# AaltoML/nonstationary-audio-gp

Measured on AMD Instinct MI355X. Metric: audio samples/sec filtered+smoothed (state dim 146, per EP sweep), higher is better.
Workload: dtype f64

## Files before the change

nonstationary-audio-gp_amd/csrc/nagp_api.hip:

```cpp
#include "nagp_inst.hpp"
#include "nagp_recon.hpp"
#include "nagp_fbsample.hpp"
#include "nagp_epsample.hpp"
#include "nagp_slowfb.hpp"
#include "nagp_nmf.hpp"
#include "nagp_pstft.hpp"
#include "nagp_segp.hpp"
#include "nagp_gppad.hpp"
#include "nagp_gppad_lap.hpp"
#include "nagp_tridiag.hpp"
#include "nagp_nmf_temp.hpp"
#include "nagp_sebf.hpp"
#include "../../include/nagp.h"

NAGP_LIST_ALL(extern template __global__)
NAGP_LIST_FBSAMPLE(extern template __global__)
NAGP_LIST_EPSAMPLE(extern template __global__)
NAGP_LIST_SLOWFB(extern template __global__)
NAGP_LIST_NMF(extern template __global__)
NAGP_LIST_PSTFT(extern template __global__)
NAGP_LIST_SEGP(extern template __global__)
NAGP_LIST_GPPAD(extern template __global__)
NAGP_LIST_GPPAD_CAS(extern template __global__)
NAGP_LIST_GPPAD_LAP(extern template __global__)
// ... 146 lines not shown
  int mfma_sp = 0;
  int big_sp = 0;
  int gain768 = 0;
  int gain_mfma = 0;
  int gain_inv = 0;
  double* d_ainv = nullptr;
  size_t gbuf_doubles = 0;
  MfmaPar mpar{};
  size_t lds_mfma = 0;
  int hph_lds = 0, sta_f = 0, sta_ep = 0, DG_f = 1, DG_ep = 1, cache_f = 0, cache_ep = 0, kb_f = 16;
  bool want_PS = false;
  bool need_PF = false;
  MomSrc src_all{};
  int src_f = 0, src_ep = 0, kb_ih = 16, chunk_cap_f = 0;
  MomSp sp{};
  int sp_ih = 0, sp_gf = 0, kb_sp = 16, hph_sp = 1; size_t lds_sp = 0;
  int sp_ep = 0; size_t lds_ep_sp = 0;
  int sq_c0 = -1, sq_ok = 0, sq_ih = 0, kb_sq = 16, hph_sq = 1; size_t lds_sq = 0; int sq_ep = 0; size_t lds_ep_sq = 0; int sq_gf = 0;
  int a8_gf = 0, a8_tpt = 1, a8_st = 0, kb_a8 = 16; size_t lds_a8 = 0;
  int seq_ih = 0;
  int sp_ih8 = 0; size_t lds_sp8 = 0;
  int place_cyc[4] = {0, 0, 0, 0};
  int qf_sp = 0;
  hipStream_t stream = nullptr;
  hipStream_t stream2 = nullptr;
  bool pipeline = false;
  int nc = 1;
  std::vector<double*> slotG, slotD;
  std::vector<char> slot_tiled;
  std::vector<int> slot_cap;
  std::vector<size_t> slot_gps;
  int n_full_slots = 0, n_recycled = 0;
  size_t mat_doubles = 0;
  size_t gstep = 0; int dpacked = 0;
  std::vector<double*> c_spanbuf, c_spanvec, c_mspanbuf, c_mspanvec;
  std::vector<double*> c_bnd, c_mbnd;
  std::vector<hipStream_t> s_apply;
  std::vector<hipEvent_t> ev_bnd, ev_app;
  ChunkTab* h_tab = nullptr;
  std::vector<double*> c_xbuf;
  unsigned long long* h_progress = nullptr;
  hipEvent_t ev_filter = nullptr, ev_s2 = nullptr;
  bool xsweep = false;
  std::vector<hipEvent_t> ev_chunk; hipEvent_t ev_red = nullptr;
  double* red_all = nullptr; double* red0 = nullptr;
  Bufs b{};
// ... 214 lines not shown
```

nonstationary-audio-gp_amd/csrc/nagp_api_plan.hpp:

```cpp

#include "nagp_msr_desc.hpp"

static void placed_lists(int CD, int nd, int c0, int npt, const std::vector<unsigned char>& code, const std::vector<int>& bd, bool place,
                         std::vector<int>& placed, int cyc[4]) {
  struct Entry { std::vector<int> placed; int cyc[4]; };
  typedef std::tuple<int, int, int, int, std::vector<unsigned char>> Key;
  static std::mutex mu;
  static std::map<Key, Entry> cache;
  if (!place) { msr_place_weights(CD, npt, bd, placed, cyc, 0); return; }
  std::lock_guard<std::mutex> lk(mu);
  const Key key(CD, nd, c0, npt, code);
  auto it = cache.find(key);
  if (it == cache.end()) {
    Entry e;
    msr_place_weights(CD, npt, bd, e.placed, e.cyc);
    it = cache.emplace(key, std::move(e)).first;
  }
  placed = it->second.placed;
  std::copy(it->second.cyc, it->second.cyc + 4, cyc);
}

static int plan_create(nagp_plan** out, int32_t B, const nagp_model* models, const nagp_ihgp_tables* tables,
                       int64_t T, const nagp_opts* o, const DevSwitches& dev) {
  if (!out || !models || !o || B < 1 || T < 1) FAIL(NAGP_EINVAL, "null/empty argument");
  *out = nullptr;
  const nagp_model& m0 = models[0];
  if (!m0.block_offsets) FAIL(NAGP_EINVAL, "problem 0: NULL block_offsets");
  if (m0.M < 1 || m0.M > MAXM) FAIL(NAGP_EUNSUPPORTED, "M=%d outside 1..%d", m0.M, MAXM);
  if (m0.S < m0.M || m0.S > 1024) FAIL(NAGP_EUNSUPPORTED, "S=%d unsupported", m0.S);
  if (o->kind != NAGP_KIND_GF_EP && o->kind != NAGP_KIND_IHGP && o->kind != NAGP_KIND_GIEKF) FAIL(NAGP_EINVAL, "kind");
  if (o->kind == NAGP_KIND_IHGP && o->mode != NAGP_MODE_PREDICT)
    FAIL(NAGP_EUNSUPPORTED, "the reference's IHGP nlml mode is broken (SURVEY C-11)");
  if (o->ep_itts < 1) FAIL(NAGP_EINVAL, "ep_itts < 1");
  const bool ekf = (o->kind == NAGP_KIND_GIEKF);
  if (!ekf) {
    if (!o->wn || !o->xn_unscaled || o->n_pts < 1 || !o->ep_damping) FAIL(NAGP_EINVAL, "cubature/damping missing");
    if (o->lik_kind == NAGP_LIK_POWER) {
      if (m0.M != 2 * m0.D || o->cub_dim != m0.D) FAIL(NAGP_EINVAL, "POWER likelihood needs M=2D, cub_dim=D");
    } else {
      if (m0.M != m0.D + m0.N || o->cub_dim != m0.N || !m0.Wnmf) FAIL(NAGP_EINVAL, "NMF likelihood needs M=D+N, cub_dim=N, Wnmf");
      const int nmax = (o->kind == NAGP_KIND_IHGP) ? MOM_MAXCD : MOM_MAXCD_GF;
      if (m0.N > nmax) FAIL(NAGP_EUNSUPPORTED, "N=%d > %d NMF components", m0.N, nmax);
// ... 449 lines not shown
      if (tq.n_grid != NG) { nagp_plan_destroy(p); FAIL(NAGP_EINVAL, "n_grid differs between problems"); }
      double* d = ht.data() + (size_t)q * tsz;
      const nagp_model& mq = models[q];
      for (int n = 0; n < sh.M; ++n) {
        const int bs = sh.bsz[n], o0 = sh.off[n];
        const double h = mq.h_val[n];
        const double* pp = tq.PPlist + tq.pp_offsets[n];
        const double* pg = tq.PGlist + tq.pg_offsets[n];
        for (int g = 0; g < NG; ++g) {
          const double* ppr = pp + (size_t)g * bs * bs;
          d[itab_hph(sh, NG) + (size_t)n * NG + g] = h * h * ppr[0];
          for (int i = 0; i < bs; ++i) d[itab_wcol(sh, NG) + ((size_t)n * NG + g) * sh.BS + i] = h * ppr[i];
          const double* pgr = pg + (size_t)g * 2 * bs * bs;
          d[itab_v(sh, NG) + (size_t)n * NG + g] = h * h * pgr[0];
          for (int i = 0; i < bs; ++i)
            for (int j = 0; j < bs; ++j)
              d[itab_g(sh, NG) + ((size_t)n * NG + g) * sh.BS * sh.BS + sh.BS * i + j] = pgr[bs * bs + i + bs * j];
        }
        d[itab_hph0(sh, NG) + n] = h * h * mq.Pinf[(size_t)o0 + (size_t)sh.S * o0];
        for (int i = 0; i < bs; ++i) d[itab_wcol0(sh, NG) + (size_t)n * sh.BS + i] = h * mq.Pinf[(size_t)(o0 + i) + (size_t)sh.S * o0];
      }
    }
    PLAN_TRY(dalloc(p, &p->d_tab, ht.size(), false));
    PLAN_TRY(dalloc(p, &p->d_r, NG, false));
    PLAN_HIP(hipMemcpyAsync(p->d_tab, ht.data(), ht.size() * sizeof(double), hipMemcpyHostToDevice, p->stream));
    PLAN_HIP(hipMemcpyAsync(p->d_r, tables[0].r_grid, (size_t)NG * sizeof(double), hipMemcpyHostToDevice, p->stream));
    PLAN_HIP(hipStreamSynchronize(p->stream));
    p->tb.NG = NG; p->tb.r = p->d_r; p->tb.base = p->d_tab;
    p->tb.lr0 = std::log10(tables[0].r_grid[0]);
    p->tb.inv_dlr = (double)(NG - 1) / (std::log10(tables[0].r_grid[NG - 1]) - p->tb.lr0);
  }

  if (o->kind == NAGP_KIND_IHGP) {
    p->NT_ih = (mom_variant(mc) >= 9) ? 512 : 256;
    p->DG_f = pick_DG(o->lik_kind, o->n_pts, p->NT_ih, sh.D, o->cub_dim);
    MomCfg t = mc; t.DG = p->DG_f; t.cache_tabs = 1; t.store_a = (o->lik_kind == NAGP_LIK_POWER_NMF_SQRT) ? 1 : 0;
    p->kb_ih = IH_KB;
    if (p->src_all.n_src >= 2 && sh.BS == 4) {
      t.src = p->src_all;
      while (p->kb_ih > 4 && ihgp_filter_lds_doubles(sh, t, p->tb.NG, 0, p->kb_ih) * sizeof(double) > 156 * 1024) p->kb_ih /= 2;
      if (ihgp_filter_lds_doubles(sh, t, p->tb.NG, 0, p->kb_ih) * sizeof(double) <= 156 * 1024) p->src_f = 1;
      else { t.src = MomSrc{}; p->kb_ih = IH_KB; }
    }
    p->hph_lds = 1;
    if (ihgp_filter_lds_doubles(sh, t, p->tb.NG, p->hph_lds, p->kb_ih) * sizeof(double) > 156 * 1024) p->hph_lds = 0;
    if (ihgp_filter_lds_doubles(sh, t, p->tb.NG, p->hph_lds, p->kb_ih) * sizeof(double) > 156 * 1024) t.store_a = 0;
    if (ihgp_filter_lds_doubles(sh, t, p->tb.NG, p->hph_lds, p->kb_ih) * sizeof(double) > 156 * 1024) t.cache_tabs = 0;
    p->cache_f = t.cache_tabs; p->sta_f = t.store_a;
    p->lds_ih = ihgp_filter_lds_doubles(sh, t, p->tb.NG, p->hph_lds, p->kb_ih) * sizeof(double);
    if (dev.stamps) fprintf(stderr, "[nagp plan] ihgp filter: LDS %zu B, hph table in LDS %d, cubature tables in LDS %d, block-structured mom %d, mom LDS %zu B, block stride %d\n", p->lds_ih, p->hph_lds, p->cache_f, p->src_f, mom_lds_doubles(t) * sizeof(double), (int)sh.BS);
    if (sh.BS == 4 && p->sp.enabled && !p->src_f && sh.M <= 64 && sh.D <= 4 * MSP_DT && o->n_pts <= MSP_NT + 64 && (o->n_pts + 3) / 4 <= MSP_NW * MSP_NST) {
      p->kb_sp = IH_KB; p->hph_sp = 1;
      auto need = [&]() { return ihgp_adf_lds_doubles(sh, o->cub_dim, p->tb.NG, p->hph_sp, p->kb_sp) * sizeof(double) + 16; };
      if (need() > 156 * 1024) p->kb_sp = 8;
      if (need() > 156 * 1024) p->hph_sp = 0;
      if (need() <= 156 * 1024) {
        p->sp_ih = 1; p->lds_sp = need();
        if (p->sp.bdesc && dev.ih_roles) {
          const int kb0 = p->kb_sp, hph0 = p->hph_sp;
          auto need8 = [&]() { return ihgp_adf8_lds_doubles(sh, o->cub_dim, p->tb.NG, p->hph_sp, p->kb_sp) * sizeof(double) + 16; };
          if (need8() > 156 * 1024) p->kb_sp = 8;
          if (need8() > 156 * 1024) p->hph_sp = 0;
          if (need8() <= 156 * 1024) { p->sp_ih8 = 1; p->lds_sp8 = need8(); }
          else { p->kb_sp = kb0; p->hph_sp = hph0; }
          if (p->sp_ih8 && dev.ih_kb && dev.ih_kb != p->kb_sp) {
            const int kb1 = p->kb_sp;
            p->kb_sp = dev.ih_kb;
            if (need8() <= 156 * 1024) p->lds_sp8 = need8(); else p->kb_sp = kb1;
          }
        }
        p->qf_sp = (p->sp_ih8 && !dev.ih_tables && o->cub_dim <= 6) ? qform_pick(sh.D, !dev.ih_qform) : QF_RUNTIME;
        PLAN_TRY(set_kernel(p->k.ih_adf, pick_ih_adf(FORM_SP, o->cub_dim, p->sp_ih8, dev.ih_tables, dev.stamps, p->qf_sp), p->sp_ih8 ? p->lds_sp8 : p->lds_sp));
      }
    }
    if (sh.BS == 4 && p->sq_ok && !p->src_f && sh.M <= 64) {
      p->kb_sq = IH_KB; p->hph_sq = 1;
      auto needq = [&]() { return ihgp_adf8sq_lds_doubles(sh, o->cub_dim, p->tb.NG, p->hph_sq, p->kb_sq) * sizeof(double) + 16; };
      if (needq() > 156 * 1024) p->kb_sq = 8;
      if (needq() > 156 * 1024) p->hph_sq = 0;
      if (needq() <= 156 * 1024) {
        p->sq_ih = 1; p->lds_sq = needq();
        PLAN_TRY(set_kernel(p->k.ih_adf, pick_ih_adf(FORM_SQ, o->cub_dim, true, false, false, QF_RUNTIME), p->lds_sq));
      }
    }
    p->seq_ih = dev.ih_seq && !p->sq_ih && !p->sp_ih && !p->src_f;
    if (dev.stamps) fprintf(stderr, "[nagp plan] ihgp ADF sweep, square-root amplitudes in the staged form: %d (LDS %zu B, ring %d steps, hph table in LDS %d)\n", p->sq_ih, p->lds_sq, p->kb_sq, p->hph_sq);
    if (dev.stamps) fprintf(stderr, "[nagp plan] ihgp ADF sweep in the sparse-point form: %d (LDS %zu B, ring %d steps, hph table in LDS %d), role-specialised waves %d (LDS %zu B), table form of stage 1b %d, Q/v form %s, weights placed %d (LDS cycles of member reads + weight stores %d + %d, second copy %d + %d), sequential kernels in every sweep %d\n", p->sp_ih, p->lds_sp, p->kb_sp, p->hph_sp, p->sp_ih8, p->lds_sp8, (int)(p->sp_ih8 && dev.ih_tables), qform_name(p->qf_sp), (int)dev.ih_place, p->place_cyc[2], p->place_cyc[3], p->place_cyc[0], p->place_cyc[1], p->seq_ih);
    PLAN_TRY(set_kernel(p->k.ih_filter, pick_ih_filter(mom_variant(mc), p->src_f, sh.BS == 8), p->lds_ih));
    for (int mode = 0; mode < 2; ++mode) {
      PLAN_TRY(set_kernel(p->k.aff_compose[mode], pick_aff_compose(mode, sh.BS), 0));
      PLAN_TRY(set_kernel(p->k.aff_boundary[mode], pick_aff_boundary(mode, sh.BS), 0));
      PLAN_TRY(set_kernel(p->k.aff_apply[mode], pick_aff_apply(mode, sh.BS), 0));
    }
    PLAN_TRY(set_kernel(p->k.ih_scan, pick_ih_scan(sh.BS), 0));
  } else {
    if (!ekf) p->DG_f = pick_DG(o->lik_kind, o->n_pts, p->NT_a, sh.D, o->cub_dim);
    MomCfg t = mc; t.DG = p->DG_f; t.cache_tabs = ekf ? 0 : 1; t.store_a = (!ekf && o->lik_kind == NAGP_LIK_POWER_NMF_SQRT) ? 1 : 0;
    if (!split && !ekf && p->sp.enabled && p->LB_a == 256 && p->NT_a == MSP_NT && sh.M <= 64 && sh.D <= 4 * MSP_DT && o->n_pts <= MSP_NT + 64 &&
        (o->n_pts + 3) / 4 <= MSP_NW * MSP_NST) {
      p->sp_gf = 1; t.sp = p->sp;
    }
    if (!split && !ekf && p->sq_ok && !p->src_all.n_src && p->LB_a == 256 && p->NT_a == 256 && sh.M <= 64) { p->sq_gf = 1; t.sq_form = 1; t.store_a = 0; }
    const size_t cap = 156 * 1024 - filter_cpl_doubles(sh) * sizeof(double);
    p->kb_f = 16;
    if (filter_lds_doubles(sh, t, ekf ? 1 : 0, p->kb_f) * sizeof(double) > cap) p->kb_f = 8;
    if (filter_lds_doubles(sh, t, ekf ? 1 : 0, p->kb_f) * sizeof(double) > cap) p->kb_f = 4;
    if (filter_lds_doubles(sh, t, ekf ? 1 : 0, p->kb_f) * sizeof(double) > cap) t.store_a = 0;
    if (filter_lds_doubles(sh, t, ekf ? 1 : 0, p->kb_f) * sizeof(double) > cap) t.cache_tabs = 0;
    if (filter_lds_doubles(sh, t, ekf ? 1 : 0, p->kb_f) * sizeof(double) > cap) p->kb_f = 2;
    if (filter_lds_doubles(sh, t, ekf ? 1 : 0, p->kb_f) * sizeof(double) > cap) p->kb_f = 1;
// ... 196 lines not shown
```

nonstationary-audio-gp_amd/csrc/nagp_ihgp.hpp:

```cpp
#pragma once
#include <type_traits>
#include "nagp_kernels.hpp"
#include "nagp_momsq.hpp"
#include "nagp_lookup.hpp"

namespace nagp {

struct IhgpTabs {
  int NG;
  const double* r;
  double lr0;
  double inv_dlr;
  const double* base;
};
__host__ __device__ inline size_t itab_hph(const Shape&, int) { return 0; }
__host__ __device__ inline size_t itab_wcol(const Shape& s, int NG) { return (size_t)s.M * NG; }
__host__ __device__ inline size_t itab_hph0(const Shape& s, int NG) { return (size_t)s.M * NG * (1 + s.BS); }
__host__ __device__ inline size_t itab_wcol0(const Shape& s, int NG) { return (size_t)s.M * NG * (1 + s.BS) + s.M; }
__host__ __device__ inline size_t itab_g(const Shape& s, int NG) { return (size_t)s.M * NG * (1 + s.BS) + (1 + s.BS) * (size_t)s.M; }
__host__ __device__ inline size_t itab_v(const Shape& s, int NG) { return itab_g(s, NG) + (size_t)s.M * NG * s.BS * s.BS; }
__host__ __device__ inline size_t itab_size(const Shape& s, int NG) { return itab_v(s, NG) + (size_t)s.M * NG; }

__device__ __forceinline__ int nearest_idx(const IhgpTabs& tb, double R) {
  if (!(R == R) || isinf(R)) return 0;
// ... 229 lines not shown
      }
      if (do_mom) lds_barrier();
      if (mc.stamps && tid == 0) { st_b = __builtin_readcyclecounter(); st[5] += st_b - st_a; st_a = st_b; }
    }
    __syncthreads();
    for (int i = tid; i < nb; i += NT) g_lZ[k0 + i] = (rZ[i] < 0.0) ? rlZ[i] : log(rZ[i]);
    for (int i = tid; i < nb * M; i += NT) {
      g_tt[(size_t)k0 * M + i] = rtt[i]; g_tn[(size_t)k0 * M + i] = rtn[i]; g_R[(size_t)k0 * M + i] = rR[i];
      g_fm[(size_t)k0 * M + i] = rfm[i];
    }
    for (int i = tid; i < nb * S; i += NT) g_MF[(size_t)k0 * S + i] = rMF[i];
    __syncthreads();
  }
  if (act && n_clamped) atomicAdd(&b.counters[(size_t)pb * 4 + 1], n_clamped);
  if (mc.stamps && tid == 0)
    for (int i = 0; i < 8; ++i) mc.stamps[i] += st[i];
}

__host__ __device__ inline size_t ihgp_adf_ring_doubles(const Shape& s, int kb) { return (size_t)kb * (8 * s.M + 3); }
__host__ __device__ inline size_t ihgp_adf_lds_doubles(const Shape& s, int CD, int NG, int hph_lds, int kb) {
  return (size_t)s.D * s.N + 2 * 68 + NG + (hph_lds ? (size_t)s.M * NG : 0) + ihgp_adf_ring_doubles(s, kb) + (s.S + 1) / 2 + 2 +
         msp_lds_doubles(CD, s.D);
}
__host__ __device__ inline size_t ihgp_adf8_lds_doubles(const Shape& s, int CD, int NG, int hph_lds, int kb) {
  return ihgp_adf_lds_doubles(s, CD, NG, hph_lds, kb) - msp_lds_doubles(CD, s.D) + msp_lds_doubles(CD, s.D, 1);
}

__device__ __forceinline__ int nearest_idx3(msp_rp r, int NG, double lr0, double inv_dlr, double rmax, double R) {
  if (!(R == R) || isinf(R)) return 0;
  if (R > rmax) {
    const double dmin = fabs(r[NG - 1] - R);
    if (fabs(r[0] - R) == dmin) return 0;
    int i = NG - 1;
    while (i > 0 && fabs(r[i - 1] - R) == dmin) --i;
    return i;
  }
  int est = 0;
  if (R > 0.0) {
    const double f = (coarse_log10(R) - lr0) * inv_dlr;
    est = (f <= 0.0) ? 0 : ((f >= (double)(NG - 1)) ? NG - 1 : (int)(f + 0.5));
  }
  const int mid = (est < 1) ? 1 : ((est > NG - 2) ? NG - 2 : est);
  const double d0 = fabs(r[mid - 1] - R), d1 = fabs(r[mid] - R), d2 = fabs(r[mid + 1] - R);
  int best = mid - 1; double bd = d0;
  if (d1 < bd) { bd = d1; best = mid; }
  if (d2 < bd) best = mid + 1;
  return best;
}
// ... 248 lines not shown
    }
    ih_ring_flush(L, G, k0, nb, M, S, tid, NT);
  }
  ih_lane_end(ln, b);
  ih_st_store(st, mc.stamps);
}

__device__ __forceinline__ void ih_window_reads(msp_rp p_rg, msp_rp p_hph, bool hph_in_lds, int mid, double& r0, double& r1, double& r2, double& h0, double& h1,
                                                double& h2) {
  r0 = p_rg[mid - 1]; r1 = p_rg[mid]; r2 = p_rg[mid + 1];
  if (hph_in_lds) { h0 = p_hph[mid - 1]; h1 = p_hph[mid]; h2 = p_hph[mid + 1]; }
}
__device__ __forceinline__ void ih_window_pick(int mid, double r0, double r1, double r2, double h0, double h1, double h2, msp_rp p_rg, msp_rp p_hph,
                                               const double* g_hph, bool hph_in_lds, double rmax, int NG, double R, int& idx, double& hph) {
  const int sel = lookup_pick3(r0, r1, r2, R);
  idx = mid - 1 + sel;
  hph = (sel == 0) ? h0 : ((sel == 1) ? h1 : h2);
  if (lookup_beyond(rmax, R)) {
    idx = lookup_tail(p_rg, NG, R);
    hph = hph_in_lds ? p_hph[idx] : g_hph[idx];
  } else if (!hph_in_lds) hph = g_hph[idx];
}

template <int CD, bool STAMPS = false, int QF = QF_RUNTIME>
__global__ void __launch_bounds__(MSR_NT) ihgp_adf8_kernel(Shape sh, Bufs b, MomCfg mc, MomSp sp, IhgpTabs tb, IhgpPar ip) {
  static_assert(CD >= 1 && CD <= 6, "the 2 x 35 outputs of Q / 2Q / v at CD = 7 do not fit the lanes of wave 0: ihgp_adf8b_kernel");
  extern __shared__ __attribute__((aligned(16))) double lds[];
  const int tid = threadIdx.x;
  const int wave = __builtin_amdgcn_readfirstlane(tid >> 6);
  constexpr int NT = MSR_NT;
  const int S = sh.S, M = sh.M, D = sh.D, NG = tb.NG, KB = ip.kb;
  const int64_t T = sh.T;
  IhLds ld;
  ih_lds_setup(ld, lds, sh, b, mc, tb, ip, CD, 0, tid, NT);
  IhRows gr;
  ih_rows(gr, sh, b);
  msr_init(CD, D, ld.ws);
  __syncthreads();
  if (wave >= MSR_W0) {
    MsrW<CD, true> xw;
    msr_setup_W<CD>(xw, mc, sp, ld.sW, ld.fmu, ld.HPH, ld.ws, false, msr_desc_p_base(), sp.bdesc + msr_desc_pos_base());
    asm volatile("" : "+v"(xw.d_qv));
    asm volatile("" : "+v"(xw.p_c[0]), "+v"(xw.p_c1[0]), "+v"(xw.p_c2[0]));
    const int wk_slot = (wave == MSR_W0 + (ip.dbg_wave & 7)) ? 8 : ((wave == MSR_W0 + MSR_NWK - 1) ? 16 : -1);
    const bool wk_stamp = STAMPS && mc.stamps && wk_slot >= 0 && (tid & 63) == 0;
    unsigned long long wk_a = 0, wk_b = 0, wk[8] = {0, 0, 0, 0, 0, 0, 0, 0};
    if (wk_stamp) wk_a = __builtin_readcyclecounter();
#define WK_STAMP(slot) do { if constexpr (STAMPS) if (wk_stamp) { wk_b = __builtin_readcyclecounter(); wk[slot] += wk_b - wk_a; wk_a = wk_b; } } while (0)
    auto wstep = [&](int kk) __attribute__((always_inline)) {
      lds_barrier();
      WK_STAMP(2);
      msr_stage1b_direct<CD, true>(xw, ld.sn2a, ld.ry[kk]);
      WK_STAMP(3);
      lds_barrier();
      WK_STAMP(4);
      msr_sums(xw);
      WK_STAMP(5);
      lds_barrier();
      WK_STAMP(7);
    };
// ... 67 lines not shown
    return;
  }
  MsrS<CD> x;
  msr_setup_S<CD>(x, mc, sp, ld.fmu, ld.HPH, ld.ws, msr_desc_p_base());
  MsrQ<CD> xq;
  MsrRT rt;
  msr_setup_Q<CD>(xq, mc, ld.sW, ld.fmu, ld.HPH, ld.ws);

  auto serial = [&](auto WV, auto LKV) __attribute__((always_inline)) {
  constexpr int WT = decltype(WV)::value, LK = decltype(LKV)::value;
  const int wave = WT;
  const int lane = tid & 63;
  IhLane ln;
  double wrow[CD];
  ih_lane_setup<CD>(ln, ld, sh, b, ip, NG, wave, lane, wrow);
  const msp_rp p_w = (msp_rp)(ld.sW + (ln.sub ? ln.n : 0) * CD);
  unsigned long long st_a = 0, st_b = 0, st[8] = {0, 0, 0, 0, 0, 0, 0, 0};
  const bool stamp = STAMPS && mc.stamps && tid == ((ip.dbg_wave & 32) ? 64 : 0);
#define IH_STAMP(slot) do { if constexpr (STAMPS) if (stamp) { st_b = __builtin_readcyclecounter(); st[slot] += st_b - st_a; st_a = st_b; } } while (0)

  double lk_lr0 = tb.lr0, lk_inv = tb.inv_dlr, lk_rmax = ld.rmax;
  int lk_ng2 = NG - 2;
  asm volatile("" : "+v"(lk_lr0), "+v"(lk_inv), "+v"(lk_rmax), "+v"(lk_ng2));
  double lk_c1, lk_c0;
  lookup_seed_consts(tb.lr0, tb.inv_dlr, lk_c1, lk_c0);
  asm volatile("" : "+v"(lk_c1), "+v"(lk_c0));
  const bool hph_in_lds = ip.hph_lds != 0;

  double hph = 0.0, wc[4] = {0, 0, 0, 0}, Am[4] = {0, 0, 0, 0}, fmun = 0.0;
  int w_mid = 1;
  double w_r0 = 0.0, w_r1 = 0.0, w_r2 = 0.0, w_h0 = 0.0, w_h1 = 0.0, w_h2 = 0.0;
  int w_idx = 0;
  auto head = [&](int64_t k, auto IN_LOOP) __attribute__((always_inline)) {
    if (ln.act) {
      if (decltype(IN_LOOP)::value || k > 0) {
        int idx;
        {
          if constexpr (!decltype(IN_LOOP)::value) {
            w_mid = lookup_mid(lk_ng2, lk_lr0, lk_inv, ln.Rprev);
            ih_window_reads(ln.p_rg, ln.p_hph, hph_in_lds, w_mid, w_r0, w_r1, w_r2, w_h0, w_h1, w_h2);
            ih_window_pick(w_mid, w_r0, w_r1, w_r2, w_h0, w_h1, w_h2, ln.p_rg, ln.p_hph, ln.g_hph, hph_in_lds, lk_rmax, lk_ng2 + 2, ln.Rprev, w_idx, hph);
          }
          idx = w_idx;
          if (stamp) { asm volatile("" :: "v"(idx), "v"(hph)); IH_STAMP(6); }
        }
        const double2* w = reinterpret_cast<const double2*>(ln.g_wcol + (size_t)idx * 4);
        const double2 w0 = w[0], w1 = w[1];
        wc[0] = w0.x; wc[1] = w0.y; wc[2] = w1.x; wc[3] = w1.y;
      } else {
        hph = ld.tab[itab_hph0(sh, NG) + ln.n];
        const double* w = ld.tab + itab_wcol0(sh, NG) + (size_t)ln.n * 4;
#pragma unroll
        for (int i = 0; i < 4; ++i) wc[i] = w[i];
      }
#pragma unroll
      for (int i = 0; i < 4; ++i) {
        double a0 = ln.A4[4 * i] * ln.mreg[0], a1 = ln.A4[4 * i + 1] * ln.mreg[1];
        a0 = fma(ln.A4[4 * i + 2], ln.mreg[2], a0); a1 = fma(ln.A4[4 * i + 3], ln.mreg[3], a1);
        Am[i] = a0 + a1;
      }
      fmun = ln.hn * Am[0];
      *ln.p_fmu = fmun; *ln.p_HPH = hph;
      if (stamp) { IH_STAMP(7); }
    }
  };
  if (stamp) st_a = __builtin_readcyclecounter();
  if (wave <= 1) head(ip.k_start, std::false_type{});
  double ls_shift = mc.link_shift;
  int qv_dlim = mc.D - (lane & 1);
  const bool ls_on = tid - 64 * x.lw >= 0 && tid - 64 * x.lw < CD * mc.nd;
  asm volatile("" : "+v"(ls_shift), "+v"(qv_dlim));
  msp_rp accp = x.accp;
  asm volatile("" : "+v"(accp));
  double pw[(WT == 0) ? CD * (CD + 1) / 2 : 1] = {0.0};
  if constexpr (WT == 0) {
    msp_wproducts<CD>(wrow, (ip.dbg_wave & 64) != 0, pw);
#pragma unroll
    for (int q = 0; q < CD * (CD + 1) / 2; ++q) asm volatile("" : "+v"(pw[q]));
  }
  auto qv_or_link = [&]() __attribute__((always_inline)) {
    msp_wave_fence();
    if (wave == 0) msr_qv_serial<CD, QF>(xq, mc, qv_dlim);
    else if constexpr (LK >= 0) msr_link_serial<CD, LK>(x, ls_on, ls_shift);
    else msp_link<CD>(x, mc);
  };
  qv_or_link();
  if (stamp) st_a = __builtin_readcyclecounter();

  auto step = [&](const int64_t k, const int kk) __attribute__((always_inline)) {
      lds_barrier();
      IH_STAMP(0);
      {
        if (wave == 1) msr_etable<CD>(x, mc);
      }
      lds_barrier();
      IH_STAMP(1);
      const int ko = kk * M;
      double wr[CD], t_old = 0.0, n_old = 0.0;
      {
        t_old = ln.p_tt[ko]; n_old = ln.p_tn[ko];
#pragma unroll
        for (int j = 0; j < CD; ++j) wr[j] = (WT == 0) ? p_w[j] : 0.0;
        msr_reduce_tab<CD>(x, rt);
      }
      lds_barrier();
      IH_STAMP(2);
      {
        msr_reduce_bins<CD>(x, rt);
        msp_wave_fence();
        if (ln.act) {
          double Z, d1, d2;
          msp_outputs_b<CD, WT == 0>(accp, ln.n - D, wr, pw, ld.pEP1, mc.jitter, Z, d1, d2);
          if (stamp) { asm volatile("" :: "v"(d2)); IH_STAMP(4); }
          const double r1 = rcp_nr(fma(d2, hph, 1.0));
          double tnew = fma(ip.w_new, -d2 * r1, ip.w_old * t_old);
          const double nnew = fma(ip.w_new, fma(-fmun, d2, d1) * r1, ip.w_old * n_old);
          if (!(tnew > 0.0)) ++ln.n_clamped;
          tnew = max0(tnew);
          {
            w_mid = lookup_mid_ttau_c(lk_ng2, lk_c1, lk_c0, tnew);
            ih_window_reads(ln.p_rg, ln.p_hph, hph_in_lds, w_mid, w_r0, w_r1, w_r2, w_h0, w_h1, w_h2);
          }
          double Rn = 1.0 / tnew;
          double g = 0.0;
          {
            double gx = fma(nnew, Rn, -fmun) * rcp_nr(hph + Rn);
            asm volatile("" : "+v"(gx));
            g = (Rn < INFINITY) ? gx : 0.0;
          }
          typedef double d2v __attribute__((ext_vector_type(2)));
          d2v m01, m23;
          ln.mreg[0] = fma(wc[0], g, Am[0]); ln.mreg[1] = fma(wc[1], g, Am[1]); ln.mreg[2] = fma(wc[2], g, Am[2]); ln.mreg[3] = fma(wc[3], g, Am[3]);
          m01.x = ln.mreg[0]; m01.y = ln.mreg[1]; m23.x = ln.mreg[2]; m23.y = ln.mreg[3];
          ih_window_pick(w_mid, w_r0, w_r1, w_r2, w_h0, w_h1, w_h2, ln.p_rg, ln.p_hph, ln.g_hph, hph_in_lds, lk_rmax, lk_ng2 + 2, Rn, w_idx, hph);
          ln.p_tt[ko] = tnew; ln.p_tn[ko] = nnew; ln.p_R[ko] = Rn;
          typedef d2v __attribute__((address_space(3))) * lds_d2p;
          lds_d2p mf = (lds_d2p)(ln.p_MF + 4 * ko);
          mf[0] = m01; mf[1] = m23;
          ln.p_fm[ko] = ln.hn * ln.mreg[0];
          ln.Rprev = Rn;
          if (ln.n == 0) ld.rZ[kk] = Z;
          if (stamp) { asm volatile("" :: "v"(ln.Rprev)); IH_STAMP(5); }
        }
        if (k + 1 < T) {
          head(k + 1, std::true_type{});
          qv_or_link(); IH_STAMP(3);
        }
      }
  };
  {
    __syncthreads();
    for (int64_t k = ip.k_start; k < T; ++k) step(k, (int)(k & (KB - 1)));
    __syncthreads();
  }
#undef IH_STAMP
  ih_lane_end(ln, b);
  if (stamp)
// ... 522 lines not shown
```

nonstationary-audio-gp_amd/csrc/nagp_lookup.hpp:

```cpp
#pragma once
#include <math.h>

#if defined(__HIPCC__)
#define NAGP_LK_HD __host__ __device__ __forceinline__
#else
#define NAGP_LK_HD inline
#endif

namespace nagp {

NAGP_LK_HD double lookup_log10(double R) {
  unsigned long long u;
  __builtin_memcpy(&u, &R, 8);
  const int e = (int)((u >> 52) & 0x7ff) - 1023;
  const unsigned long long mu = (u & 0x000fffffffffffffull) | 0x3ff0000000000000ull;
  double t;
  __builtin_memcpy(&t, &mu, 8);
  t -= 1.0;
  return ((double)e + t + 0.3466 * t * (1.0 - t)) * 0.30102999566398120;
}

NAGP_LK_HD bool lookup_beyond(double rmax, double R) { return R > rmax && R < INFINITY; }
template <class P>
NAGP_LK_HD int lookup_tail(P r, int NG, double R) {
// ... 36 lines not shown
NAGP_LK_HD int lookup_pick3(double r0, double r1, double r2, double R) {
  const double d0 = fabs(r0 - R), d1 = fabs(r1 - R), d2 = fabs(r2 - R);
  int s = 0; double bd = d0;
  if (d1 < bd) { bd = d1; s = 1; }
  if (d2 < bd) s = 2;
  return s;
}

template <class P>
NAGP_LK_HD int nearest_idx3_sl(P r, int NG, double lr0, double inv_dlr, double rmax, double R) {
  if (lookup_beyond(rmax, R)) return lookup_tail(r, NG, R);
  const int mid = lookup_mid(NG - 2, lr0, inv_dlr, R);
  return mid - 1 + lookup_pick3(r[mid - 1], r[mid], r[mid + 1], R);
}
template <class P>
NAGP_LK_HD int nearest_idx3_seeded(P r, int NG, double lr0, double inv_dlr, double rmax, double ttau) {
  const int mid = lookup_mid_ttau(NG - 2, lr0, inv_dlr, ttau);
  const double r0 = r[mid - 1], r1 = r[mid], r2 = r[mid + 1];
  const double R = 1.0 / ttau;
  if (lookup_beyond(rmax, R)) return lookup_tail(r, NG, R);
  return mid - 1 + lookup_pick3(r0, r1, r2, R);
}

}
```

nonstationary-audio-gp_amd/csrc/nagp_momsp.hpp:

```cpp
#pragma once
#include "nagp_dev.hpp"
#include "nagp_qform.hpp"
#include "nagp_msr_desc.hpp"

namespace nagp {

constexpr int MSP_NT = 256;
constexpr int MSP_NPS = 2;
constexpr int MSP_DT = 16;
constexpr int MSP_MAXCD = 7;

typedef const double __attribute__((address_space(3))) * msp_rp;
typedef double __attribute__((address_space(3))) * msp_wp;


__host__ __device__ inline size_t msp_lds_doubles(int CD, int D, int LAY = 0) { return (size_t)msp_layout(CD, D, LAY).total; }

__device__ __forceinline__ double rcp_nr(double x) {
  double r = __builtin_amdgcn_rcp(x);
  double e = fma(-x, r, 1.0); r = fma(r, e, r);
  e = fma(-x, r, 1.0); r = fma(r, e, r);
  return r;
}
__device__ __forceinline__ int opaque_zero() { int z = 0; asm volatile("" : "+v"(z)); return z; }
// ... 487 lines not shown
  }
  asm volatile("" : "+v"(Zs));
#pragma unroll
  for (int q = 0; q < NR; ++q) asm volatile("" : "+v"(av[q]));
  Z = pEP * __builtin_fmax(Zs, jitter);
  const double Zinv = pEP * rcp_nr(Z);
  double s1, s2;
  if constexpr (SUB) {
    double a0 = 0.0, a1 = 0.0;
#pragma unroll
    for (int j = 0; j < CD; ++j) { if (j & 1) a1 = fma(wrow[j], av[j], a1); else a0 = fma(wrow[j], av[j], a0); }
    s1 = a0 + a1;
    double b0 = 0.0, b1 = 0.0;
#pragma unroll
    for (int q = 0; q < nq; ++q) { if (q & 1) b1 = fma(pw[q], av[CD + q], b1); else b0 = fma(pw[q], av[CD + q], b0); }
    s2 = b0 + b1;
  } else {
    s1 = av[0]; s2 = av[1];
  }
  d1 = Zinv * s1;
  d2 = fma(-d1, d1, Zinv * s2);
}

constexpr int MSR_NT = 512;
constexpr int MSR_W0 = 2;

template <int CD>
struct MsrS {
  int lw;
  double xdc; msp_rp a_mu, a_s2, a_l0[CD], a_l0own, a_qrow, a_qjj, a_v; msp_wp a_out;
  msp_rp r_p[MSR_RW]; msp_wp r_dst; msp_rp accp;
};
template <int CD, bool PL = false>
struct MsrW {
  static constexpr int NPS = 1, CS = MSR_CS;
  static constexpr bool PLACED = PL;
  int q_kind; msp_rp q_ww, q_src; msp_wp q_out0, q_out1, q_out2, q_out3;
  int b_kind; msp_rp b_p0, b_p1, b_p2;
  msp_rp p_e[1][MSP_NZ], p_q[1][6]; msp_wp p_c[1], p_c1[1], p_c2[1]; double p_wn[1]; bool p_ok[1]; int p_any[1];
  msp_rp d_lk[CD], d_qv;
  msp_rp s_mem[MSR_NMEM]; msp_wp s_out; int s_grp;
  msp_rp t_bin[MSR_KT], t_fa[MSR_KT], t_fb[MSR_KT]; msp_wp t_out; int t_grp;
};

__device__ __forceinline__ void msr_init(int CD, int D, double* ws) {
  const MspLay l = msp_layout(CD, D, 1);
// ... 338 lines not shown
```

Measured before the change: 1.458 million.

## Replace grid lookup with precomputed ttau thresholds and split wave-0 output sums across half-waves

On the host, bisection over double bit patterns produces exact ttau thresholds for the nearest-grid lookup and integer seed constants, then checks that they reproduce the reference index. The per-step lookup in the ADF8 kernel becomes an integer multiply-shift seed plus two threshold compares, with no reciprocal needed to select the index. The gain expression is also rewritten in terms of ttau. Separately, wave 0 splits the s1/s2 quadratic-form reduction between its two 32-lane halves and exchanges partial sums with permlane32_swap. The cost is extra LDS for the threshold tail and host-side search time at plan creation. The ADF8 path is now gated on the thresholds being proved.

Result: faster. 1.510 million (median of 6 runs) (+3.6%).

```diff
diff --git a/nonstationary-audio-gp_amd/csrc/nagp_api.hip b/nonstationary-audio-gp_amd/csrc/nagp_api.hip
--- a/nonstationary-audio-gp_amd/csrc/nagp_api.hip
+++ b/nonstationary-audio-gp_amd/csrc/nagp_api.hip
@@ -192,6 +192,7 @@
   int sp_ih8 = 0; size_t lds_sp8 = 0;
   int place_cyc[4] = {0, 0, 0, 0};
   int qf_sp = 0;
+  int thr_ok = 0; double thr_us = 0.0;
   hipStream_t stream = nullptr;
   hipStream_t stream2 = nullptr;
   bool pipeline = false;
diff --git a/nonstationary-audio-gp_amd/csrc/nagp_api_plan.hpp b/nonstationary-audio-gp_amd/csrc/nagp_api_plan.hpp
--- a/nonstationary-audio-gp_amd/csrc/nagp_api_plan.hpp
+++ b/nonstationary-audio-gp_amd/csrc/nagp_api_plan.hpp
@@ -18,6 +18,26 @@
   }
   placed = it->second.placed;
   std::copy(it->second.cyc, it->second.cyc + 4, cyc);
+}
+
+static bool grid_thresholds(const double* r, int NG, double lr0, double inv_dlr, std::vector<double>& ext, double& us) {
+  struct Entry { std::vector<double> ext; bool ok; };
+  static std::mutex mu;
+  static std::map<std::vector<double>, Entry> cache;
+  std::lock_guard<std::mutex> lk(mu);
+  const std::vector<double> key(r, r + NG);
+  us = 0.0;
+  auto it = cache.find(key);
+  if (it == cache.end()) {
+    Entry e;
+    e.ext.resize((size_t)lookup_thr_doubles(NG));
+    const auto t0 = std::chrono::steady_clock::now();
+    e.ok = lookup_thresholds(r, NG, lr0, inv_dlr, e.ext.data());
+    us = std::chrono::duration<double, std::micro>(std::chrono::steady_clock::now() - t0).count();
+    it = cache.emplace(key, std::move(e)).first;
+  }
+  ext = it->second.ext;
+  return it->second.ok;
 }
 
 static int plan_create(nagp_plan** out, int32_t B, const nagp_model* models, const nagp_ihgp_tables* tables,
@@ -513,13 +533,17 @@
       }
     }
     PLAN_TRY(dalloc(p, &p->d_tab, ht.size(), false));
-    PLAN_TRY(dalloc(p, &p->d_r, NG, false));
-    PLAN_HIP(hipMemcpyAsync(p->d_tab, ht.data(), ht.size() * sizeof(double), hipMemcpyHostToDevice, p->stream));
-    PLAN_HIP(hipMemcpyAsync(p->d_r, tables[0].r_grid, (size_t)NG * sizeof(double), hipMemcpyHostToDevice, p->stream));
-    PLAN_HIP(hipStreamSynchronize(p->stream));
-    p->tb.NG = NG; p->tb.r = p->d_r; p->tb.base = p->d_tab;
+    p->tb.NG = NG; p->tb.base = p->d_tab;
     p->tb.lr0 = std::log10(tables[0].r_grid[0]);
     p->tb.inv_dlr = (double)(NG - 1) / (std::log10(tables[0].r_grid[NG - 1]) - p->tb.lr0);
+    std::vector<double> hr(tables[0].r_grid, tables[0].r_grid + NG), ext;
+    p->thr_ok = grid_thresholds(tables[0].r_grid, NG, p->tb.lr0, p->tb.inv_dlr, ext, p->thr_us) ? 1 : 0;
+    hr.insert(hr.end(), ext.begin(), ext.end());
+    PLAN_TRY(dalloc(p, &p->d_r, hr.size(), false));
+    PLAN_HIP(hipMemcpyAsync(p->d_tab, ht.data(), ht.size() * sizeof(double), hipMemcpyHostToDevice, p->stream));
+    PLAN_HIP(hipMemcpyAsync(p->d_r, hr.data(), hr.size() * sizeof(double), hipMemcpyHostToDevice, p->stream));
+    PLAN_HIP(hipStreamSynchronize(p->stream));
+    p->tb.r = p->d_r;
   }
 
   if (o->kind == NAGP_KIND_IHGP) {
@@ -547,7 +571,7 @@
       if (need() > 156 * 1024) p->hph_sp = 0;
       if (need() <= 156 * 1024) {
         p->sp_ih = 1; p->lds_sp = need();
-        if (p->sp.bdesc && dev.ih_roles) {
+        if (p->sp.bdesc && dev.ih_roles && (p->thr_ok || dev.ih_tables || o->cub_dim > 6)) {
           const int kb0 = p->kb_sp, hph0 = p->hph_sp;
           auto need8 = [&]() { return ihgp_adf8_lds_doubles(sh, o->cub_dim, p->tb.NG, p->hph_sp, p->kb_sp) * sizeof(double) + 16; };
           if (need8() > 156 * 1024) p->kb_sp = 8;
@@ -576,7 +600,7 @@
     }
     p->seq_ih = dev.ih_seq && !p->sq_ih && !p->sp_ih && !p->src_f;
     if (dev.stamps) fprintf(stderr, "[nagp plan] ihgp ADF sweep, square-root amplitudes in the staged form: %d (LDS %zu B, ring %d steps, hph table in LDS %d)\n", p->sq_ih, p->lds_sq, p->kb_sq, p->hph_sq);
-    if (dev.stamps) fprintf(stderr, "[nagp plan] ihgp ADF sweep in the sparse-point form: %d (LDS %zu B, ring %d steps, hph table in LDS %d), role-specialised waves %d (LDS %zu B), table form of stage 1b %d, Q/v form %s, weights placed %d (LDS cycles of member reads + weight stores %d + %d, second copy %d + %d), sequential kernels in every sweep %d\n", p->sp_ih, p->lds_sp, p->kb_sp, p->hph_sp, p->sp_ih8, p->lds_sp8, (int)(p->sp_ih8 && dev.ih_tables), qform_name(p->qf_sp), (int)dev.ih_place, p->place_cyc[2], p->place_cyc[3], p->place_cyc[0], p->place_cyc[1], p->seq_ih);
+    if (dev.stamps) fprintf(stderr, "[nagp plan] ihgp ADF sweep in the sparse-point form: %d (LDS %zu B, ring %d steps, hph table in LDS %d), role-specialised waves %d (LDS %zu B), table form of stage 1b %d, Q/v form %s, weights placed %d (LDS cycles of member reads + weight stores %d + %d, second copy %d + %d), look-up thresholds proved %d (searched in %.0f us), sequential kernels in every sweep %d\n", p->sp_ih, p->lds_sp, p->kb_sp, p->hph_sp, p->sp_ih8, p->lds_sp8, (int)(p->sp_ih8 && dev.ih_tables), qform_name(p->qf_sp), (int)dev.ih_place, p->place_cyc[2], p->place_cyc[3], p->place_cyc[0], p->place_cyc[1], p->thr_ok, p->thr_us, p->seq_ih);
     PLAN_TRY(set_kernel(p->k.ih_filter, pick_ih_filter(mom_variant(mc), p->src_f, sh.BS == 8), p->lds_ih));
     for (int mode = 0; mode < 2; ++mode) {
       PLAN_TRY(set_kernel(p->k.aff_compose[mode], pick_aff_compose(mode, sh.BS), 0));
diff --git a/nonstationary-audio-gp_amd/csrc/nagp_ihgp.hpp b/nonstationary-audio-gp_amd/csrc/nagp_ihgp.hpp
--- a/nonstationary-audio-gp_amd/csrc/nagp_ihgp.hpp
+++ b/nonstationary-audio-gp_amd/csrc/nagp_ihgp.hpp
@@ -275,8 +275,9 @@
   return (size_t)s.D * s.N + 2 * 68 + NG + (hph_lds ? (size_t)s.M * NG : 0) + ihgp_adf_ring_doubles(s, kb) + (s.S + 1) / 2 + 2 +
          msp_lds_doubles(CD, s.D);
 }
+__host__ __device__ inline int ih_thr_tail(int NG) { return NG + (NG & 1); }
 __host__ __device__ inline size_t ihgp_adf8_lds_doubles(const Shape& s, int CD, int NG, int hph_lds, int kb) {
-  return ihgp_adf_lds_doubles(s, CD, NG, hph_lds, kb) - msp_lds_doubles(CD, s.D) + msp_lds_doubles(CD, s.D, 1);
+  return ihgp_adf_lds_doubles(s, CD, NG, hph_lds, kb) - msp_lds_doubles(CD, s.D) + msp_lds_doubles(CD, s.D, 1) + ih_thr_tail(NG);
 }
 
 __device__ __forceinline__ int nearest_idx3(msp_rp r, int NG, double lr0, double inv_dlr, double rmax, double R) {
@@ -571,6 +572,24 @@
   } else if (!hph_in_lds) hph = g_hph[idx];
 }
 
+__device__ __forceinline__ void ih_thr_reads(msp_rp p_thr, msp_rp p_hph, bool hph_in_lds, int mid, double& ta, double& tb, double& h0, double& h1, double& h2) {
+  ta = p_thr[mid - 1]; tb = p_thr[mid];
+  if (hph_in_lds) { h0 = p_hph[mid - 1]; h1 = p_hph[mid]; h2 = p_hph[mid + 1]; }
+}
+__device__ __forceinline__ void ih_thr_pick(int mid, double ta, double tb, double h0, double h1, double h2, double h_first, msp_rp p_rg, msp_rp p_hph,
+                                            const double* g_hph, bool hph_in_lds, double t_beyond, double t_inf, int NG, double ttau, double R, int& idx,
+                                            double& hph) {
+  const int sel = lookup_pick_thr(ta, tb, ttau);
+  const bool at_inf = ttau <= t_inf;
+  idx = at_inf ? 0 : mid - 1 + sel;
+  hph = (sel == 0) ? h0 : ((sel == 1) ? h1 : h2);
+  hph = at_inf ? h_first : hph;
+  if (ttau <= t_beyond && !at_inf) {
+    idx = lookup_tail(p_rg, NG, R);
+    hph = hph_in_lds ? p_hph[idx] : g_hph[idx];
+  } else if (!hph_in_lds && !at_inf) hph = g_hph[idx];
+}
+
 template <int CD, bool STAMPS = false, int QF = QF_RUNTIME>
 __global__ void __launch_bounds__(MSR_NT) ihgp_adf8_kernel(Shape sh, Bufs b, MomCfg mc, MomSp sp, IhgpTabs tb, IhgpPar ip) {
   static_assert(CD >= 1 && CD <= 6, "the 2 x 35 outputs of Q / 2Q / v at CD = 7 do not fit the lanes of wave 0: ihgp_adf8b_kernel");
@@ -581,10 +600,11 @@
   const int S = sh.S, M = sh.M, D = sh.D, NG = tb.NG, KB = ip.kb;
   const int64_t T = sh.T;
   IhLds ld;
-  ih_lds_setup(ld, lds, sh, b, mc, tb, ip, CD, 0, tid, NT);
+  ih_lds_setup(ld, lds, sh, b, mc, tb, ip, CD, ih_thr_tail(NG), tid, NT);
   IhRows gr;
   ih_rows(gr, sh, b);
   msr_init(CD, D, ld.ws);
+  for (int i = tid; i < NG - 1; i += NT) ld.tail[i] = tb.r[NG + i];
   __syncthreads();
   if (wave >= MSR_W0) {
     MsrW<CD, true> xw;
@@ -698,10 +718,13 @@
   double lk_lr0 = tb.lr0, lk_inv = tb.inv_dlr, lk_rmax = ld.rmax;
   int lk_ng2 = NG - 2;
   asm volatile("" : "+v"(lk_lr0), "+v"(lk_inv), "+v"(lk_rmax), "+v"(lk_ng2));
-  double lk_c1, lk_c0;
-  lookup_seed_consts(tb.lr0, tb.inv_dlr, lk_c1, lk_c0);
-  asm volatile("" : "+v"(lk_c1), "+v"(lk_c0));
+  double lk_tbey = tb.r[2 * NG - 1], lk_tinf = tb.r[2 * NG];
+  unsigned int lk_c1 = (unsigned int)tb.r[2 * NG + 1]; int lk_c0 = (int)tb.r[2 * NG + 2];
+  asm volatile("" : "+v"(lk_tbey), "+v"(lk_tinf), "+v"(lk_c1), "+v"(lk_c0));
+  const msp_rp p_thr = (msp_rp)ld.tail + opaque_zero();
   const bool hph_in_lds = ip.hph_lds != 0;
+  double lk_h0 = hph_in_lds ? ln.p_hph[0] : ln.g_hph[0];
+  asm volatile("" : "+v"(lk_h0));
 
   double hph = 0.0, wc[4] = {0, 0, 0, 0}, Am[4] = {0, 0, 0, 0}, fmun = 0.0;
   int w_mid = 1;
@@ -748,11 +771,31 @@
   asm volatile("" : "+v"(ls_shift), "+v"(qv_dlim));
   msp_rp accp = x.accp;
   asm volatile("" : "+v"(accp));
+  constexpr int HALF_CT = (QF == QF_K4 || QF == QF_K8) ? 1 : ((QF == QF_K16P) ? 0 : -1);
+  int half_s = (D <= 32) ? 1 : 0;
+  if constexpr (HALF_CT < 0) {
+    asm volatile("" : "+v"(half_s));
+    half_s = __builtin_amdgcn_readfirstlane(half_s);
+  }
+  const bool half = (WT == 0) && ((HALF_CT >= 0) ? (HALF_CT == 1) : (half_s != 0));
+  const bool upper = lane >= 32;
+  msp_rp accp_h = accp;
   double pw[(WT == 0) ? CD * (CD + 1) / 2 : 1] = {0.0};
   if constexpr (WT == 0) {
-    msp_wproducts<CD>(wrow, (ip.dbg_wave & 64) != 0, pw);
+    if (half) {
+      const int hd = lane & 31;
+      double wh[CD];
+#pragma unroll
+      for (int j = 0; j < CD; ++j) wh[j] = (hd < D) ? ld.sW[hd * CD + j] : 0.0;
+      msp_wproducts<CD>(wh, (ip.dbg_wave & 64) != 0, pw);
+      msp_half_coeffs<CD>(wh, upper, pw);
+      accp_h = accp + (upper ? msp_half_terms<CD>() : 0);
+    } else {
+      msp_wproducts<CD>(wrow, (ip.dbg_wave & 64) != 0, pw);
+    }
 #pragma unroll
     for (int q = 0; q < CD * (CD + 1) / 2; ++q) asm volatile("" : "+v"(pw[q]));
+    asm volatile("" : "+v"(accp_h));
   }
   auto qv_or_link = [&]() __attribute__((always_inline)) {
     msp_wave_fence();
@@ -776,7 +819,7 @@
       {
         t_old = ln.p_tt[ko]; n_old = ln.p_tn[ko];
 #pragma unroll
-        for (int j = 0; j < CD; ++j) wr[j] = (WT == 0) ? p_w[j] : 0.0;
+        for (int j = 0; j < CD; ++j) wr[j] = (WT == 0 && !half) ? p_w[j] : 0.0;
         msr_reduce_tab<CD>(x, rt);
       }
       lds_barrier();
@@ -784,9 +827,12 @@
       {
         msr_reduce_bins<CD>(x, rt);
         msp_wave_fence();
+        double Z = 0.0, d1 = 0.0, d2 = 0.0;
+        if constexpr (WT == 0) {
+          if (half) msp_outputs_h<CD>(accp, accp_h, pw, upper, ld.pEP1, mc.jitter, Z, d1, d2);
+        }
         if (ln.act) {
-          double Z, d1, d2;
-          msp_outputs_b<CD, WT == 0>(accp, ln.n - D, wr, pw, ld.pEP1, mc.jitter, Z, d1, d2);
+          if (!(WT == 0 && half)) msp_outputs_b<CD, WT == 0>(accp, ln.n - D, wr, pw, ld.pEP1, mc.jitter, Z, d1, d2);
           if (stamp) { asm volatile("" :: "v"(d2)); IH_STAMP(4); }
           const double r1 = rcp_nr(fma(d2, hph, 1.0));
           double tnew = fma(ip.w_new, -d2 * r1, ip.w_old * t_old);
@@ -794,21 +840,21 @@
           if (!(tnew > 0.0)) ++ln.n_clamped;
           tnew = max0(tnew);
           {
-            w_mid = lookup_mid_ttau_c(lk_ng2, lk_c1, lk_c0, tnew);
-            ih_window_reads(ln.p_rg, ln.p_hph, hph_in_lds, w_mid, w_r0, w_r1, w_r2, w_h0, w_h1, w_h2);
+            w_mid = lookup_mid_bits(lk_ng2, lk_c1, lk_c0, tnew);
+            ih_thr_reads(p_thr, ln.p_hph, hph_in_lds, w_mid, w_r0, w_r1, w_h0, w_h1, w_h2);
           }
           double Rn = 1.0 / tnew;
           double g = 0.0;
           {
-            double gx = fma(nnew, Rn, -fmun) * rcp_nr(hph + Rn);
+            double gx = fma(-fmun, tnew, nnew) * rcp_nr(fma(hph, tnew, 1.0));
             asm volatile("" : "+v"(gx));
-            g = (Rn < INFINITY) ? gx : 0.0;
+            g = (tnew > lk_tinf) ? gx : 0.0;
           }
           typedef double d2v __attribute__((ext_vector_type(2)));
           d2v m01, m23;
           ln.mreg[0] = fma(wc[0], g, Am[0]); ln.mreg[1] = fma(wc[1], g, Am[1]); ln.mreg[2] = fma(wc[2], g, Am[2]); ln.mreg[3] = fma(wc[3], g, Am[3]);
           m01.x = ln.mreg[0]; m01.y = ln.mreg[1]; m23.x = ln.mreg[2]; m23.y = ln.mreg[3];
-          ih_window_pick(w_mid, w_r0, w_r1, w_r2, w_h0, w_h1, w_h2, ln.p_rg, ln.p_hph, ln.g_hph, hph_in_lds, lk_rmax, lk_ng2 + 2, Rn, w_idx, hph);
+          ih_thr_pick(w_mid, w_r0, w_r1, w_h0, w_h1, w_h2, lk_h0, ln.p_rg, ln.p_hph, ln.g_hph, hph_in_lds, lk_tbey, lk_tinf, lk_ng2 + 2, tnew, Rn, w_idx, hph);
           ln.p_tt[ko] = tnew; ln.p_tn[ko] = nnew; ln.p_R[ko] = Rn;
           typedef d2v __attribute__((address_space(3))) * lds_d2p;
           lds_d2p mf = (lds_d2p)(ln.p_MF + 4 * ko);
diff --git a/nonstationary-audio-gp_amd/csrc/nagp_lookup.hpp b/nonstationary-audio-gp_amd/csrc/nagp_lookup.hpp
--- a/nonstationary-audio-gp_amd/csrc/nagp_lookup.hpp
+++ b/nonstationary-audio-gp_amd/csrc/nagp_lookup.hpp
@@ -1,5 +1,6 @@
 #pragma once
 #include <math.h>
+#include <vector>
 
 #if defined(__HIPCC__)
 #define NAGP_LK_HD __host__ __device__ __forceinline__
@@ -82,4 +83,92 @@
   return mid - 1 + lookup_pick3(r0, r1, r2, R);
 }
 
+#define NAGP_LOOKUP_SEED_SHIFT 8
+NAGP_LK_HD int lookup_mid_bits(int ng2, unsigned int c1, int c0, double ttau) {
+  unsigned long long u;
+  __builtin_memcpy(&u, &ttau, 8);
+  const unsigned int hi = (unsigned int)(u >> 32);
+  const int est = (c0 - (int)(unsigned int)(((unsigned long long)hi * c1) >> 32)) >> NAGP_LOOKUP_SEED_SHIFT;
+  return est < 1 ? 1 : (est > ng2 ? ng2 : est);
 }
+NAGP_LK_HD int lookup_pick_thr(double ta, double tb, double ttau) { return (int)(ttau <= ta) + (int)(ttau <= tb); }
+
+NAGP_LK_HD int lookup_thr_doubles(int NG) { return NG + 3; }
+
+template <class P>
+NAGP_LK_HD int nearest_idx3_thr(P r, P ext, int NG, double ttau) {
+  const double t_beyond = ext[NG - 1], t_inf = ext[NG];
+  const int mid = lookup_mid_bits(NG - 2, (unsigned int)ext[NG + 1], (int)ext[NG + 2], ttau);
+  int idx = mid - 1 + lookup_pick_thr(ext[mid - 1], ext[mid], ttau);
+  idx = (ttau <= t_inf) ? 0 : idx;
+  if (ttau <= t_beyond && ttau > t_inf) idx = lookup_tail(r, NG, 1.0 / ttau);
+  return idx;
+}
+
+inline double lookup_from_bits(unsigned long long u) { double x; __builtin_memcpy(&x, &u, 8); return x; }
+inline unsigned long long lookup_to_bits(double x) { unsigned long long u; __builtin_memcpy(&u, &x, 8); return u; }
+template <class F>
+inline unsigned long long lookup_bisect(unsigned long long lo, unsigned long long hi, F pred) {
+  while (hi - lo > 1) {
+    const unsigned long long m = lo + (hi - lo) / 2;
+    if (pred(m)) lo = m; else hi = m;
+  }
+  return lo;
+}
+inline bool lookup_seed_bits_consts(double lr0, double inv_dlr, unsigned int& c1, int& c0) {
+  const double a = 0.30102999566398120 * inv_dlr;
+  if (!(a > 0.0) || !(a < 2048.0) || !(fabs(lr0 * inv_dlr) < 1e6)) return false;
+  const double one = (double)(1 << NAGP_LOOKUP_SEED_SHIFT);
+  c1 = (unsigned int)floor(a * one * 4096.0 + 0.5);
+  const double z = ((1023.0 - 0.0430) * a - lr0 * inv_dlr + 0.5) * one;
+  if (!(fabs(z) < 1.0e9)) return false;
+  c0 = (int)floor(z + 0.5);
+  return true;
+}
+template <class P>
+inline bool lookup_thresholds(P r, int NG, double lr0, double inv_dlr, double* out) {
+  for (int i = 0; i < lookup_thr_doubles(NG); ++i) out[i] = 0.0;
+  if (NG < 3) return false;
+  const double rmax = r[NG - 1];
+  if (!(rmax > 0.0) || !(rmax < INFINITY)) return false;
+  const unsigned long long b_one = lookup_to_bits(1.0), b_inf = lookup_to_bits(INFINITY);
+  auto recip = [](unsigned long long u) { volatile double t = lookup_from_bits(u); return 1.0 / t; };
+  auto index = [&](unsigned long long u) { volatile double t = lookup_from_bits(u); return nearest_idx3_seeded(r, NG, lr0, inv_dlr, rmax, t); };
+  const unsigned long long b_tinf = lookup_bisect(0ull, b_one, [&](unsigned long long u) { return !(recip(u) < INFINITY); });
+  const unsigned long long b_tbey = lookup_bisect(b_tinf, b_inf, [&](unsigned long long u) { return recip(u) > rmax; });
+  const unsigned long long b_lo = b_tbey + 1;
+  if (b_lo >= b_inf || index(b_lo) != NG - 1 || index(b_inf) != 0) return false;
+  unsigned long long hi = b_inf;
+  std::vector<unsigned long long> tau((size_t)NG - 1);
+  for (int i = 0; i < NG - 1; ++i) {
+    if (index(hi) >= i + 1) return false;
+    tau[i] = lookup_bisect(b_lo, hi, [&](unsigned long long u) { return index(u) >= i + 1; });
+    hi = tau[i] + 1;
+    out[i] = lookup_from_bits(tau[i]);
+  }
+  out[NG - 1] = lookup_from_bits(b_tbey); out[NG] = lookup_from_bits(b_tinf);
+  unsigned int c1; int c0;
+  if (!lookup_seed_bits_consts(lr0, inv_dlr, c1, c0)) return false;
+  out[NG + 1] = (double)c1; out[NG + 2] = (double)c0;
+  const int ng2 = NG - 2;
+  auto seed = [&](unsigned long long u) { return lookup_mid_bits(ng2, c1, c0, lookup_from_bits(u)); };
+  auto holds = [&](unsigned long long u) {
+    if (u < b_lo || u > b_inf) return true;
+    const double t = lookup_from_bits(u);
+    int idx = 0;
+    while (idx < NG - 1 && t <= out[idx]) ++idx;
+    const int mid = seed(u);
+    return idx >= mid - 1 && idx <= mid + 1 && idx == mid - 1 + lookup_pick_thr(out[mid - 1], out[mid], t);
+  };
+  if (!holds(b_lo) || !holds(b_inf)) return false;
+  for (int i = 0; i < NG - 1; ++i)
+    if (!holds(tau[i]) || !holds(tau[i] + 1)) return false;
+  if (seed(b_lo) < seed(b_inf)) return false;
+  for (int v = seed(b_inf) + 1; v <= seed(b_lo); ++v) {
+    const unsigned long long s = lookup_bisect(b_lo, b_inf, [&](unsigned long long u) { return seed(u) >= v; });
+    if (!holds(s) || !holds(s + 1)) return false;
+  }
+  return true;
+}
+
+}
diff --git a/nonstationary-audio-gp_amd/csrc/nagp_momsp.hpp b/nonstationary-audio-gp_amd/csrc/nagp_momsp.hpp
--- a/nonstationary-audio-gp_amd/csrc/nagp_momsp.hpp
+++ b/nonstationary-audio-gp_amd/csrc/nagp_momsp.hpp
@@ -533,6 +533,55 @@
   d2 = fma(-d1, d1, Zinv * s2);
 }
 
+template <int CD>
+__host__ __device__ constexpr int msp_half_terms() { return (CD + CD * (CD + 1) / 2 + 1) / 2; }
+template <int CD>
+__device__ __forceinline__ void msp_half_coeffs(const double* wrow, bool upper, double* pw ) {
+  constexpr int nq = CD * (CD + 1) / 2, NT = CD + nq, NL = msp_half_terms<CD>();
+  double c[NT];
+#pragma unroll
+  for (int j = 0; j < CD; ++j) c[j] = wrow[j];
+#pragma unroll
+  for (int q = 0; q < nq; ++q) c[CD + q] = pw[q];
+#pragma unroll
+  for (int i = 0; i < nq; ++i) pw[i] = (i < NL) ? (upper ? ((NL + i < NT) ? c[NL + i] : 0.0) : c[i]) : 0.0;
+}
+template <int CD>
+__device__ __forceinline__ void msp_outputs_h(msp_rp acc, msp_rp acc_lane, const double* hc, bool upper, double pEP, double jitter, double& Z, double& d1, double& d2) {
+  constexpr int nq = CD * (CD + 1) / 2, NT = CD + nq, NL = msp_half_terms<CD>();
+  static_assert(NL >= CD && NL <= nq, "the lower half holds all of s1; the coefficients fit the registers of the products");
+  double av[NL];
+  double Zs = acc[3 * CD + nq];
+#pragma unroll
+  for (int i = 0; i < NL; ++i) av[i] = acc_lane[i];
+  asm volatile("" : "+v"(Zs));
+#pragma unroll
+  for (int i = 0; i < NL; ++i) asm volatile("" : "+v"(av[i]));
+  if constexpr ((NT & 1) != 0) av[NL - 1] = upper ? 0.0 : av[NL - 1];
+  Z = pEP * __builtin_fmax(Zs, jitter);
+  const double Zinv = pEP * rcp_nr(Z);
+  double a0 = 0.0, a1 = 0.0;
+#pragma unroll
+  for (int j = 0; j < CD; ++j) { if (j & 1) a1 = fma(hc[j], av[j], a1); else a0 = fma(hc[j], av[j], a0); }
+  const double pa = a0 + a1;
+  double b0 = 0.0, b1 = 0.0;
+#pragma unroll
+  for (int i = CD; i < NL; ++i) { if (i & 1) b1 = fma(hc[i], av[i], b1); else b0 = fma(hc[i], av[i], b0); }
+  const double pb = b0 + b1;
+  const double t = pa + pb;
+  typedef unsigned int u2v __attribute__((ext_vector_type(2)));
+  unsigned long long tb;
+  __builtin_memcpy(&tb, &t, 8);
+  const unsigned int tlo = (unsigned int)tb, thi = (unsigned int)(tb >> 32);
+  const u2v slo = __builtin_amdgcn_permlane32_swap(tlo, tlo, false, false), shi = __builtin_amdgcn_permlane32_swap(thi, thi, false, false);
+  const unsigned long long ub = ((unsigned long long)shi.y << 32) | slo.y;
+  double tu;
+  __builtin_memcpy(&tu, &ub, 8);
+  const double s1 = pa, s2 = pb + tu;
+  d1 = Zinv * s1;
+  d2 = fma(-d1, d1, Zinv * s2);
+}
+
 constexpr int MSR_NT = 512;
 constexpr int MSR_W0 = 2;
 
```
